# CobayaSampler/cobaya

Measured on AMD Instinct MI355X. Metric: log-posterior evals/sec (whole node), 30-dim gaussian_mixture, higher is better.
Workload: dtype f64

## Files before the change

cobaya_amd/csrc/capi.hip:

```cpp
#include "ctx.h"
#include "host_linalg.h"

int block_slots(const mcmc_hip_ctx* h, int which)
{
    if (!h->blocked) return h->d;
    int L = 0;
    for (size_t b = 0; b < h->blk_size.size(); ++b) {
        if (which == 0) L += h->blk_over[b] * h->blk_size[b];
        else if (which == 1) L += ((int)b <= h->drag_last_slow) ? h->blk_size[b] : 0;
        else L += ((int)b > h->drag_last_slow) ? h->blk_size[b] : 0;
    }
    return L;
}

int upload_constants(mcmc_hip_ctx* h)
{
    if (!h->have_prior || !h->have_target) return MCMC_HIP_OK;
    const int d = h->d, K = h->K;
    const ConstLayout cl{d, K};
    std::vector<double> c((size_t)cl.size() + 16, 0.0);
    for (int i = 0; i < d; ++i) {
        c[cl.lo() + i] = h->lo[i];
        c[cl.hi() + i] = h->hi[i];
        c[cl.loc() + i] = h->loc[i];
// ... 47 lines not shown
        if (K > 0) HIP_TRY(h, h->y.resize((size_t)K * d * h->W));
        if (K > 1) HIP_TRY(h, h->amode.resize((size_t)K * h->W));
        h->amode_valid = false;
        std::vector<double> pr((size_t)5 * dpad, 0.0);
        for (int i = 0; i < dpad; ++i) {
            pr[i] = i < d ? h->lo[i] : -INFINITY;
            pr[dpad + i] = i < d ? h->hi[i] : INFINITY;
            pr[2 * dpad + i] = i < d ? h->loc[i] : 0.0;
            const bool nrm = i < d && h->kind[i] == 1;
            pr[3 * dpad + i] = nrm ? 1.0 / h->scale[i] : 0.0;
            pr[4 * dpad + i] = nrm ? h->mls[i] : 0.0;
        }
        HIP_TRY(h, h->inc_prior.resize(pr.size()));
        HIP_TRY(h, hipMemcpyAsync(h->inc_prior.p, pr.data(), sizeof(double) * pr.size(),
                                  hipMemcpyHostToDevice, h->stream));
        if (K > 0) {
            HIP_TRY(h, h->inc_Lrow.resize((size_t)K * d * d));
            HIP_TRY(h, hipMemcpyAsync(h->inc_Lrow.p, h->Linv.data(), sizeof(double) * K * d * d,
                                      hipMemcpyHostToDevice, h->stream));
            HIP_TRY(h, h->inc_mean.resize((size_t)K * d));
            HIP_TRY(h, hipMemcpyAsync(h->inc_mean.p, h->mean.data(), sizeof(double) * K * d,
                                      hipMemcpyHostToDevice, h->stream));
        }
        h->y_valid = false; h->amode_valid = false;
    }
    HIP_TRY(h, hipStreamSynchronize(h->stream));
    return MCMC_HIP_OK;
}

namespace {

int lds_check(mcmc_hip_ctx* h)
{
    if (h->kb || h->huge) return MCMC_HIP_OK;
    const size_t lds = mcmc::step_lds_bytes(h->K, 256, h->gs, mcmc::v_slab(h->d));
    if (lds > mcmc::kLdsMax)
        return fail(h, MCMC_HIP_ERR_ARG,
                    "the step kernel needs %zu bytes of LDS per workgroup (> 160 KiB): fewer "
                    "mixture modes or a smaller group_size are required", lds);
    return MCMC_HIP_OK;
}

int set_target_common(mcmc_hip_ctx* h, int K, const double* means, const double* covs,
                      const double* weights, bool normalized)
{
    const int d = h->d;
    if (K < 1 || K > mcmc::kMaxModes)
// ... 193 lines not shown
        acc(h->nrows.resize(W));
    }
    acc(hipHostMalloc((void**)&h->pin_mom, sizeof(double) * (G * d + np + 2),
                      hipHostMallocCoherent | hipHostMallocMapped));
    if (h->pin_mom) acc(hipHostGetDevicePointer((void**)&h->pin_mom_dev, h->pin_mom, 0));
    acc(hipHostMalloc((void**)&h->pin_T, sizeof(double) * 4 * d * d, hipHostMallocDefault));
    for (auto& e : h->pin_T_done) acc(hipEventCreateWithFlags(&e, hipEventDisableTiming));
    acc(hipEventCreateWithFlags(&h->mom_event, hipEventDisableTiming));
    if (h->incremental) {
        int prio_least = 0, prio_greatest = 0;
        acc(hipDeviceGetStreamPriorityRange(&prio_least, &prio_greatest));
        acc(hipStreamCreateWithPriority(&h->stream2, hipStreamNonBlocking, prio_least));
        acc(hipEventCreateWithFlags(&h->mark, hipEventDisableTiming));
        acc(hipEventCreateWithFlags(&h->T_event, hipEventDisableTiming));
        if (const char* e = getenv("MCMC_HIP_EAGER_DIRECTIONS")) h->lazy_dirs = !(e[0] && e[0] != '0');
        if (const char* e = getenv("MCMC_HIP_LOOKAHEAD")) h->lookahead = std::max(1, atoi(e));
        if (const char* e = getenv("MCMC_HIP_DUO")) h->duo = (e[0] && e[0] != '0') ? 1 : 0;
        if (const char* e = getenv("MCMC_HIP_ACCEPT_SLACK")) {
            const double v = strtod(e, nullptr);
            h->accept_slack = v < mcmc::kAcceptSlack ? mcmc::kAcceptSlack : v;
        }
        for (auto& D : h->dirs) acc(hipEventCreateWithFlags(&D.ready, hipEventDisableTiming));
        h->prefetch = !getenv("MCMC_HIP_NO_PREFETCH");
    }
    if (r == hipSuccess) r = hipMemsetAsync(h->gsum.p, 0, sizeof(double) * G * d, h->stream);
    if (r == hipSuccess) r = hipMemsetAsync(h->pooled.p, 0, sizeof(double) * np, h->stream);
    if (r == hipSuccess) r = hipMemsetAsync(h->dshift.p, 0, sizeof(double) * d, h->stream);
    if (r == hipSuccess) r = hipMemsetAsync(h->stuck.p, 0, sizeof(int), h->stream);
    if (r == hipSuccess) r = hipMemsetAsync(h->acc_total.p, 0, sizeof(unsigned long long), h->stream);
    if (r == hipSuccess) r = hipStreamSynchronize(h->stream);
    if (r != hipSuccess) {
        fail(nullptr, MCMC_HIP_ERR_DEVICE, "device allocation failed: %s", hipGetErrorString(r));
        mcmc_hip_destroy(h);
        return MCMC_HIP_ERR_DEVICE;
    }
    *out = h;
    return MCMC_HIP_OK;
}

void mcmc_hip_destroy(mcmc_hip_ctx* h)
{
    if (!h) return;
    (void)hipSetDevice(h->cfg.device);
    if (h->stream) (void)hipStreamSynchronize(h->stream);
    if (h->stream2) (void)hipStreamSynchronize(h->stream2);
    resolve_timing(h);
// ... 11 lines not shown
    h->cblock.release(); h->dT.release(); h->V.release(); h->rows.release(); h->gsum.release();
    h->Sg.release(); h->pooled.p = nullptr;  h->dshift.release(); h->ex.release(); h->elp.release();
    h->ell.release(); h->eder.release(); h->escratch.release(); h->dLrow.release();
    h->dLcol.release(); h->weight_i.release(); h->prej.release();
    h->burn.release(); h->stuck.release(); h->nrows.release(); h->nacc.release();
    h->acc_total.p = nullptr;
    h->dblk.release(); h->vflag.release(); h->vflag_f.release(); h->Vf.release(); h->drag_cs.release();
    for (auto& sl : h->slots)
        if (sl.p) (void)hipHostFree(sl.p);
    h->ck.ring.release(); h->ck.wsum.release(); h->ck.payload.release(); h->ck.ws.release();
    h->ck.out.release(); h->ck.acc_prev.release();
    h->bd.ring.release(); h->bd.bounds.release(); h->bd.payload.release();
    if (h->bd.pin) (void)hipHostFree(h->bd.pin);
    if (h->ck.pin_out) (void)hipHostFree(h->ck.pin_out);
    destroy_product(h->mg); destroy_product(h->ac); destroy_product(h->bf);
    destroy_product(h->evd); destroy_product(h->dv); destroy_product(h->imp);
    h->imp.hist.destroy();
    if (h->ck.ev) (void)hipEventDestroy(h->ck.ev);
    if (h->pin_mom) (void)hipHostFree(h->pin_mom);
    if (h->pin_T) (void)hipHostFree(h->pin_T);
    for (auto& e : h->pin_T_done) if (e) (void)hipEventDestroy(e);
    if (h->mom_event) (void)hipEventDestroy(h->mom_event);
    h->pack_out.release(); h->pack_off.release();
    h->y.release(); h->amode.release(); h->inc_prior.release(); h->inc_Lrow.release();
    h->inc_mean.release();
    {
        auto& B = h->bg;
        B.bjs.release(); B.es.release(); B.Afused.release();
        B.resp.release(); B.theta0.release(); B.Astream.release(); B.weights.release();
        B.X.release(); B.dbins.release(); B.delta.release(); B.trial.release(); B.lp_t.release();
        B.Ea.release(); B.psum.release(); B.epsum.release(); B.edelta.release(); B.etrial.release(); B.elp.release();
        B.echi2.release(); B.ecl.release(); B.eA.release();
    }
    h->fnt.points.release(); h->fnt.lp_t.release(); h->fnt.Ea.release(); h->fnt.ll_t.release();
    h->fnt.bad.release();
    h->mv.q.release();
    h->fnt.dinputs.release(); h->fnt.ll_new.release(); h->fnt.ll_c.release();
    h->fnt.epts.release(); h->fnt.ell.release();
    for (auto& b : h->fnt.pts) b.release();
    if (h->stream) (void)hipStreamDestroy(h->stream);
    delete h;
}

int mcmc_hip_set_prior(mcmc_hip_ctx* h, const int32_t* kind, const double* a, const double* b,
                       const int32_t* periodic)
{
    if (!h) return MCMC_HIP_ERR_ARG;
// ... 327 lines not shown
    HIP_TRY(h, hipMemcpyAsync(h->logpost.p, lpost.data(), sizeof(double) * W, hipMemcpyHostToDevice, s));
    HIP_TRY(h, hipMemcpyAsync(h->logprior.p, lp.data(), sizeof(double) * W, hipMemcpyHostToDevice, s));
    HIP_TRY(h, hipMemcpyAsync(h->loglike.p, ll.data(), sizeof(double) * W, hipMemcpyHostToDevice, s));
    HIP_TRY(h, hipMemcpyAsync(h->weight_i.p, ones.data(), sizeof(int) * W, hipMemcpyHostToDevice, s));
    HIP_TRY(h, hipMemcpyAsync(h->prej.p, zeros.data(), sizeof(int) * W, hipMemcpyHostToDevice, s));
    HIP_TRY(h, hipMemcpyAsync(h->burn.p, burn.data(), sizeof(int) * W, hipMemcpyHostToDevice, s));
    HIP_TRY(h, hipMemcpyAsync(h->nacc.p, z64.data(), sizeof(long long) * W, hipMemcpyHostToDevice, s));
    if (h->nrows.p)
        HIP_TRY(h, hipMemcpyAsync(h->nrows.p, zeros.data(), sizeof(int) * W, hipMemcpyHostToDevice, s));
    HIP_TRY(h, hipMemsetAsync(h->stuck.p, 0, sizeof(int), s));
    if (h->fnt.bad.p) HIP_TRY(h, hipMemsetAsync(h->fnt.bad.p, 0, sizeof(int), s));
    if (h->fnt.on && h->fnt.n_fn > 0) {
        auto& F = h->fnt;
        if (F.last_eval_n != (int)W) return fail(h, MCMC_HIP_ERR_STATE, "no component log-likelihoods of the state");
        HIP_TRY(h, hipMemcpyAsync(F.ll_c.p, F.last_eval.data(), sizeof(double) * F.n_fn * W, hipMemcpyHostToDevice, s));
        F.llc_valid = true;
    }
    HIP_TRY(h, hipMemsetAsync(h->acc_total.p, 0, sizeof(unsigned long long), s));
    if (h->thin_acc.p) HIP_TRY(h, hipMemsetAsync(h->thin_acc.p, 0, sizeof(int) * W, s));
    HIP_TRY(h, hipStreamSynchronize(s));
    h->step = 0;
    h->have_state = true;
    h->mv.checked = false; h->mv.broken = false;
    h->y_valid = false; h->amode_valid = false;
    return MCMC_HIP_OK;
}

int mcmc_hip_get_state(mcmc_hip_ctx* h, double* x, double* logpost, double* logprior,
                       double* loglike, int32_t* weight)
{
    if (!h) return MCMC_HIP_ERR_ARG;
    if (!h->have_state) return fail(h, MCMC_HIP_ERR_STATE, "no state: call set_state first");
    const size_t W = h->W, d = h->d;
    hipStream_t s = h->stream;
    HIP_TRY(h, hipSetDevice(h->cfg.device));
    std::vector<double> xt;
    if (x) {
        xt.resize(W * d);
        HIP_TRY(h, hipMemcpyAsync(xt.data(), h->x.p, sizeof(double) * W * d, hipMemcpyDeviceToHost, s));
    }
    if (logpost) HIP_TRY(h, hipMemcpyAsync(logpost, h->logpost.p, sizeof(double) * W, hipMemcpyDeviceToHost, s));
    if (logprior) HIP_TRY(h, hipMemcpyAsync(logprior, h->logprior.p, sizeof(double) * W, hipMemcpyDeviceToHost, s));
    if (loglike) HIP_TRY(h, hipMemcpyAsync(loglike, h->loglike.p, sizeof(double) * W, hipMemcpyDeviceToHost, s));
    if (weight) HIP_TRY(h, hipMemcpyAsync(weight, h->weight_i.p, sizeof(int) * W, hipMemcpyDeviceToHost, s));
    HIP_TRY(h, hipStreamSynchronize(s));
    if (x)
        for (size_t w = 0; w < W; ++w)
// ... 38 lines not shown
            return fail(h, MCMC_HIP_ERR_ARG, "walker %zu has a non-finite log-posterior", w);
        for (size_t i = 0; i < d; ++i) xt[i * W + w] = x[w * d + i];
    }
    HIP_TRY(h, hipMemcpy(h->x.p, xt.data(), sizeof(double) * W * d, hipMemcpyHostToDevice));
    HIP_TRY(h, hipMemcpy(h->logpost.p, logpost, sizeof(double) * W, hipMemcpyHostToDevice));
    HIP_TRY(h, hipMemcpy(h->logprior.p, logprior, sizeof(double) * W, hipMemcpyHostToDevice));
    HIP_TRY(h, hipMemcpy(h->loglike.p, loglike, sizeof(double) * W, hipMemcpyHostToDevice));
    HIP_TRY(h, hipMemcpy(h->weight_i.p, weight, sizeof(int) * W, hipMemcpyHostToDevice));
    HIP_TRY(h, hipMemcpy(h->prej.p, prior_rej, sizeof(int) * W, hipMemcpyHostToDevice));
    HIP_TRY(h, hipMemcpy(h->burn.p, burn_left, sizeof(int) * W, hipMemcpyHostToDevice));
    HIP_TRY(h, hipMemcpy(h->nacc.p, n_accept, sizeof(int64_t) * W, hipMemcpyHostToDevice));
    if (h->nrows.p) HIP_TRY(h, hipMemset(h->nrows.p, 0, sizeof(int) * W));
    HIP_TRY(h, hipMemset(h->stuck.p, 0, sizeof(int)));
    if (h->fnt.bad.p) HIP_TRY(h, hipMemset(h->fnt.bad.p, 0, sizeof(int)));
    h->fnt.llc_valid = false;
    {
        unsigned long long tot = 0;
        for (size_t w = 0; w < W; ++w) tot += (unsigned long long)n_accept[w];
        HIP_TRY(h, hipMemcpy(h->acc_total.p, &tot, sizeof tot, hipMemcpyHostToDevice));
    }
    h->step = step;
    h->have_state = true;
    h->mv.checked = false; h->mv.broken = false;
    h->y_valid = false; h->amode_valid = false;
    return MCMC_HIP_OK;
}

namespace {
mcmc::ScratchShape scratch_shape_of(mcmc_hip_ctx* h)
{
    mcmc::ScratchShape s;
    const bool drag = h->drag_last_slow >= 0;
    s.d = h->d; s.K = h->K; s.W = h->W; s.group_size = h->gs;
    s.any_normal = h->norm_mask4[0] || h->norm_mask4[1] || h->norm_mask4[2] || h->norm_mask4[3];
    s.any_periodic = h->any_periodic;
    s.emit = h->cfg.emit_capacity > 0; s.emit_thin = h->emit_thin > 1;
    s.unit_t = h->cfg.temperature == 1.0;
    s.own_basis = h->own_basis; s.blocked = h->blocked;
    s.n_drag = drag ? h->drag_steps : 0;
    s.cps = block_slots(h, drag ? 1 : 0);
    s.cps_f = drag ? block_slots(h, 2) : 0;
    s.lane_compiled = h->k != nullptr; s.big_dp = h->kb ? h->kb->dp : 0; s.pair_compiled = h->kp != nullptr;
    return s;
}
}

int mcmc_hip_scratch_choice(const mcmc_hip_scratch_shape* shape, mcmc_hip_scratch_answer* out)
// ... 202 lines not shown
    HIP_TRY(h, hipSetDevice(h->cfg.device));
    HIP_TRY(h, hipMemcpyAsync(h->dshift.p, h->shift.data(), sizeof(double) * h->d,
                              hipMemcpyHostToDevice, h->stream));
    if (changed && h->ac.ro.on()) {
        h->ac.held = h->ac.head = 0;
        std::fill(h->ac.n_pairs.begin(), h->ac.n_pairs.end(), (int64_t)0);
        HIP_TRY(h, hipMemsetAsync(h->ac.ro.slab, 0, h->ac.ro.bytes(), h->stream));
    }
    HIP_TRY(h, hipStreamSynchronize(h->stream));
    return MCMC_HIP_OK;
}

int mcmc_hip_accumulate_moments(mcmc_hip_ctx* h)
{
    if (!h) return MCMC_HIP_ERR_ARG;
    if (!h->have_state) return fail(h, MCMC_HIP_ERR_STATE, "no state");
    HIP_TRY(h, hipSetDevice(h->cfg.device));
    Timed t(h, 2);
    mcmc::MomentArgs a{};
    a.x = h->x.p; a.shift = h->dshift.p; a.group_sum = h->gsum.p; a.Sg = h->Sg.p;
    a.pooled = h->pooled.p; a.W = h->W; a.G = h->G;
    if (h->huge) HIP_TRY(h, mcmc_hip_launch_huge_moments(&a, h->gs, h->d, h->stream));
    else if (h->kb) HIP_TRY(h, h->kb->moments(a, h->gs, h->d, h->stream));
    else HIP_TRY(h, h->k->moments(a, h->gs, h->stream));
    h->n_snapshots += 1;
    return MCMC_HIP_OK;
}

int mcmc_hip_read_moments(mcmc_hip_ctx* h, int64_t* n_snapshots, double* group_sum,
                          double* pooled_S, int32_t reset)
{
    if (!h) return MCMC_HIP_ERR_ARG;
    HIP_TRY(h, hipSetDevice(h->cfg.device));
    HIP_TRY(h, hipStreamSynchronize(h->stream));
    if (h->stream2) HIP_TRY(h, hipStreamSynchronize(h->stream2));
    resolve_timing(h);
    const size_t d = h->d, G = h->G, np = d * (d + 1) / 2;
    if (n_snapshots) *n_snapshots = h->n_snapshots;
    if (group_sum)
        HIP_TRY(h, hipMemcpy(group_sum, h->gsum.p, sizeof(double) * G * d, hipMemcpyDeviceToHost));
    if (pooled_S) {
        std::vector<double> p(np);
        HIP_TRY(h, hipMemcpy(p.data(), h->pooled.p, sizeof(double) * np, hipMemcpyDeviceToHost));
        for (size_t i = 0; i < d; ++i)
            for (size_t j = 0; j <= i; ++j)
                pooled_S[i * d + j] = pooled_S[j * d + i] = p[i * (i + 1) / 2 + j];
    }
// ... 136 lines not shown
```

cobaya_amd/csrc/capi_incremental.hip:

```cpp
#include "ctx.h"

int blocked_basis(mcmc_hip_ctx* h, int which, unsigned long long c0, int ncyc, int L, size_t slab,
                  DevBuf<double>& V, DevBuf<int>& flag, bool& any_1d, hipStream_t st, bool shared_schedule)
{
    if (!st) st = h->stream;
    const int nb = (int)h->blk_size.size();
    any_1d = false;
    for (int b = 0; b < nb; ++b) {
        const bool in_seq = which == 0 || (which == 1) == (b <= h->drag_last_slow);
        any_1d = any_1d || (in_seq && h->blk_size[b] == 1);
    }
    HIP_TRY(h, V.resize((size_t)h->BG * ncyc * slab));
    if (any_1d) HIP_TRY(h, flag.resize((size_t)h->BG * ncyc * L));
    mcmc::BlockedBasisArgs b{};
    b.T = h->dT.p; b.V = V.p; b.vflag = any_1d ? flag.p : nullptr;
    b.block_size = h->dblk.p; b.oversample = h->dblk.p + nb; b.i_of_j = h->dblk.p + 2 * nb;
    b.n_blocks = nb; b.d = h->d; b.which = which; b.drag_last_slow = h->drag_last_slow;
    b.L = L; b.slab = (int)slab;
    b.ld = h->d;
    b.nmax = *std::max_element(h->blk_size.begin(), h->blk_size.end());
    b.group0 = h->cfg.walker_offset / (uint32_t)h->bgs;
    b.cycle0 = (uint32_t)c0;
    b.key0 = (uint32_t)h->cfg.seed; b.key1 = (uint32_t)(h->cfg.seed >> 32);
    b.ncyc = ncyc;
// ... 282 lines not shown
    if (hit) return MCMC_HIP_OK;
    if (h->prefetch && h->lazy_dirs && h->mark_valid && h->stream2) {
        HIP_TRY(h, hipStreamWaitEvent(h->stream2, h->mark, 0));
        if (h->T_fresh) HIP_TRY(h, hipStreamWaitEvent(h->stream2, h->T_event, 0));
        const int rc = make_directions(h, C, P, span, D, h->stream2);
        if (rc != MCMC_HIP_OK) return rc;
        wait_ready = true;
    } else {
        const int rc = make_directions(h, C, P, span, D, h->stream);
        if (rc != MCMC_HIP_OK) return rc;
    }
    h->T_fresh = false;
    return MCMC_HIP_OK;
}

int launch_segment(mcmc_hip_ctx* h, const IncChoice& C, const IncPlan& P, mcmc_hip_ctx::DirSet& D,
                   bool inside, int room, bool& wait_ready, int& n)
{
    bool anchor = false;
    bool refresh_in_kernel = false;
    if (!h->y_valid || h->step % P.R == 0) {
        if (C.fold && inside) {
            refresh_in_kernel = true;
        } else {
            HIP_TRY(h, mcmc_hip_launch_whiten_state(h->x.p, h->y.p, h->inc_mean.p, h->inc_Lrow.p,
                                                    P.d, h->W, P.K, h->stream));
        }
        h->y_valid = true;
        anchor = true;
    }
    if (C.carry_modes && !h->amode_valid) anchor = true;
    n = plan_segment(P, h->step, room).n;
    if (wait_ready) {
        HIP_TRY(h, hipStreamWaitEvent(h->stream, D.ready, 0));
        wait_ready = false;
    }
    {
        Timed t(h, 0);
        const mcmc::IncStepArgs a =
            fill_inc_args(h, C, P, D, n, (anchor ? 1 : 0) | (refresh_in_kernel ? 2 : 0));
        if (C.carry_modes) h->amode_valid = true;
        HIP_TRY(h, P.launch(&a, h->stream));
        h->n_step_launches += 1;
        take_noted_kernel(h);
    }
    h->step += (unsigned long long)n;
    return MCMC_HIP_OK;
}

int prepare_next_set(mcmc_hip_ctx* h, const IncChoice& C, const IncPlan& P, int left, int n_steps)
{
    auto& N = h->dirs[h->dir_cur ^ 1];
    if (C.fold) {
// ... 54 lines not shown
    int left = n_steps;
    while (left > 0) {
        IncSeg span = plan_span(C, P, h->step, left);
        bool wait_ready = false;
        int rc = acquire_direction_set(h, C, P, span, false, wait_ready);
        if (rc != MCMC_HIP_OK) return rc;
        int n = 0;
        rc = launch_segment(h, C, P, h->dirs[h->dir_cur], false, span.n, wait_ready, n);
        if (rc != MCMC_HIP_OK) return rc;
        left -= n;
        rc = prepare_next_set(h, C, P, left, n_steps);
        if (rc != MCMC_HIP_OK) return rc;
    }
    return MCMC_HIP_OK;
}

}

mcmc::IncChoice inc_choice_of(const mcmc_hip_ctx* h)
{
    if (!h->incremental) return IncChoice{};
    const IncShape s = inc_shape_of(h);
    return mcmc::inc_choose(s, inc_any_fits(s, true));
}

int step_incremental(mcmc_hip_ctx* h, int n_steps)
{
    const int d = h->d, K = h->K;
    const IncShape S = inc_shape_of(h);
    const IncChoice C = mcmc::inc_choose(S, inc_any_fits(S, true));
    if (C.reason == mcmc::kIncBadShape || C.reason == mcmc::kIncDragShape)
        return fail(h, MCMC_HIP_ERR_ARG,
                    "incremental evaluation with dragging serves one Gaussian mode with "
                    "non-periodic priors; use evaluation: full for this model");
    if (C.reason == mcmc::kIncAnyLds)
        return fail(h, MCMC_HIP_ERR_ARG,
                    "incremental evaluation: %d modes at d=%d with %d periodic parameters do not "
                    "fit the LDS of a CU; use evaluation: full for this model", K, d, S.n_periodic);
    if (C.reason == mcmc::kIncEmitDrag && h->emit_thin > 1)
        return fail(h, MCMC_HIP_ERR_ARG,
                    "emit_thin: rows are thinned on the device by the incremental Metropolis kernels; "
                    "thin on the host");
    if (C.reason == mcmc::kIncEmitDrag)
        return fail(h, MCMC_HIP_ERR_ARG,
                    "incremental evaluation emits rows (emit_capacity > 0) with Metropolis "
                    "steps; use evaluation: full for dragging with emitted rows");
// ... 62 lines not shown
        h->y_valid = true;
    }
    HIP_TRY(h, hipStreamSynchronize(h->stream));
    const size_t W = h->W, d = (size_t)h->d * (size_t)h->K;
    std::vector<double> yt(W * d);
    HIP_TRY(h, hipMemcpy(yt.data(), h->y.p, sizeof(double) * W * d, hipMemcpyDeviceToHost));
    for (size_t w = 0; w < W; ++w)
        for (size_t i = 0; i < d; ++i) y[w * d + i] = yt[i * W + w];
    return MCMC_HIP_OK;
}

int mcmc_hip_set_whitened(mcmc_hip_ctx* h, const double* y)
{
    if (!h) return MCMC_HIP_ERR_ARG;
    if (!h->incremental || !y) return fail(h, MCMC_HIP_ERR_ARG, "not in incremental mode, or null");
    if (!h->have_state) return fail(h, MCMC_HIP_ERR_STATE, "set_full_state must precede set_whitened");
    HIP_TRY(h, hipSetDevice(h->cfg.device));
    HIP_TRY(h, hipStreamSynchronize(h->stream));
    const size_t W = h->W, d = (size_t)h->d * (size_t)h->K;
    std::vector<double> yt(W * d);
    for (size_t w = 0; w < W; ++w)
        for (size_t i = 0; i < d; ++i) yt[i * W + w] = y[w * d + i];
    HIP_TRY(h, hipMemcpy(h->y.p, yt.data(), sizeof(double) * W * d, hipMemcpyHostToDevice));
    h->y_valid = true;
    return MCMC_HIP_OK;
}

int mcmc_hip_incremental_carries_periodic(const mcmc_hip_ctx* h)
{
    return h && inc_choice_of(h).carry_periodic ? 1 : 0;
}

int mcmc_hip_accept_estimate_error(double* max_err, uint32_t* ka_at_max)
{
    if (!max_err || !ka_at_max) return MCMC_HIP_ERR_ARG;
    if (!mcmc_hip_launch_accept_estimate_error) return MCMC_HIP_ERR_ARG;
    constexpr int nb = 4096;
    double* derr = nullptr;
    uint32_t* dka = nullptr;
    std::vector<double> err(nb);
    std::vector<uint32_t> ka(nb);
    hipError_t r = hipMalloc(&derr, sizeof(double) * nb);
    if (r == hipSuccess) r = hipMalloc(&dka, sizeof(uint32_t) * nb);
    if (r == hipSuccess) r = mcmc_hip_launch_accept_estimate_error(derr, dka, nb, nullptr);
    if (r == hipSuccess) r = hipMemcpy(err.data(), derr, sizeof(double) * nb, hipMemcpyDeviceToHost);
    if (r == hipSuccess) r = hipMemcpy(ka.data(), dka, sizeof(uint32_t) * nb, hipMemcpyDeviceToHost);
    if (derr) (void)hipFree(derr);
// ... 52 lines not shown
```

cobaya_amd/csrc/ctx.h:

```cpp
#pragma once
#include "../../include/mcmc_hip.h"

#include <algorithm>
#include <cmath>
#include <cstdarg>
#include <cstdio>
#include <cstring>
#include <limits>
#include <string>
#include <vector>

#define MCMC_HIP_HOST_SIDE 1
#include "kernels.h"
#include "huge_args.h"
#include "pliklite_args.h"
#include "function_args.h"
#include "stretch_args.h"
#include "ensemble_move_args.h"
#include "checkpoint_args.h"
#include "marginal_args.h"
#include "autocorr_args.h"
#include "bestfit_args.h"
#include "evidence_args.h"
#include "derived_args.h"
// ... 112 lines not shown
    bool have_prior = false, have_target = false, have_cov = false, have_state = false;
    std::vector<int32_t> kind, periodic;
    std::vector<double> lo, hi, loc, scale, mls;
    double uniform_logp = 0.0;
    uint32_t norm_mask = 0, periodic_mask = 0;
    uint32_t norm_mask4[4] = {0, 0, 0, 0};
    bool any_periodic = false;
    std::vector<double> mean, Linv, cnorm, weight;
    std::vector<double> cov, T;
    bool blocked = false;
    std::vector<int32_t> blk_size, blk_over, i_of_j;
    int drag_last_slow = -1, drag_steps = 0;
    DevBuf<int> dblk, vflag, vflag_f;
    DevBuf<double> Vf;
    DevBuf<double> drag_cs;
    std::vector<double> shift;
    DevBuf<double> x, logpost, logprior, loglike, cblock, dT, V, rows, gsum, Sg, pooled, dshift;
    DevBuf<double> ex, elp, ell, eder, escratch, dLrow, dLcol;
    bool incremental = false;
    bool y_valid = false;
    bool own_basis = false;
    int bgs = 0, BG = 0;
    DevBuf<double> y, inc_prior, inc_Lrow, inc_mean;
    DevBuf<double> amode;
    bool amode_valid = false;
    struct DirSet {
        DevBuf<double> V, Vf, VU;
        DevBuf<int> vflag, vflag_f, colflag;
        bool has_flags = false;
        DevBuf<double> UU;
        DevBuf<double> VW, NL;
        hipEvent_t ready = nullptr;
        bool ahead = false;
        unsigned long long step0 = ~0ull, epoch = 0;
        int n = 0;
    } dirs[2];
    int dir_cur = 0;
    unsigned long long dir_epoch = 0;
    hipStream_t stream2 = nullptr;
    hipEvent_t mark = nullptr;
    bool mark_valid = false;
    bool prefetch = true;
    bool lazy_dirs = true;
    int lookahead = 4;
    size_t dir_budget = 0;
    int duo = -1;
// ... 349 lines not shown
int step_functions(mcmc_hip_ctx* h, int n_steps);
int functions_evaluate(mcmc_hip_ctx* h, int n, const double* x, double* comps);
int evaluate_binned_points(mcmc_hip_ctx* h, int n, const double* x, double* logprior, double* loglike);
int function_call(mcmc_hip_ctx* h, int n, const double* points, double* loglike);
int function_target_error(mcmc_hip_ctx* h, int bad);
inline uint32_t philox_w0(uint32_t k0, uint32_t k1, uint32_t c0, uint32_t c1, uint32_t c2, uint32_t c3)
{
    for (int r = 0; r < 10; ++r) {
        const uint64_t p0 = (uint64_t)0xD2511F53u * c0, p1 = (uint64_t)0xCD9E8D57u * c2;
        const uint32_t n0 = (uint32_t)(p1 >> 32) ^ c1 ^ k0, n2 = (uint32_t)(p0 >> 32) ^ c3 ^ k1;
        c0 = n0; c1 = (uint32_t)p1; c2 = n2; c3 = (uint32_t)p0;
        k0 += 0x9E3779B9u; k1 += 0xBB67AE85u;
    }
    return c0;
}

int step_stretch(mcmc_hip_ctx* h, int n_steps);
int blocked_basis(mcmc_hip_ctx* h, int which, unsigned long long c0, int ncyc, int L, size_t slab,
                  DevBuf<double>& V, DevBuf<int>& flag, bool& any_1d, hipStream_t st = nullptr,
                  bool shared_schedule = false);
int step_huge(mcmc_hip_ctx* h, int n_steps);
int step_incremental(mcmc_hip_ctx* h, int n_steps);
mcmc::IncChoice inc_choice_of(const mcmc_hip_ctx* h);
```

cobaya_amd/csrc/incremental_kernels.hip:

```cpp
#include <string>

#include "incremental_common.h"

#ifndef MCMC_INC_DMA_HIDDEN
#define MCMC_INC_DMA_HIDDEN(dq, mode) ((dq) >= 25 && (mode) == 0)
#endif

namespace mcmc {
namespace {

__host__ __device__ constexpr bool inc_one_wave_regs(int dq, int mode, bool per)
{
    return !per && ((mode == 1 && dq >= 31) || (mode == 2 && dq >= 32));
}

__host__ __device__ constexpr int inc_min_waves(int dq, int mode, bool per = false)
{
    if (per) return MCMC_EXP_WAVES(STEP, dq <= 8 ? 4 : dq <= 31 ? 2 : 1);
    return MCMC_EXP_WAVES(STEP,
        mode == 0 ? (dq <= 12 ? 4 : dq <= 30 ? 2 : 1)
        : mode == 1 ? ((dq <= 8 || dq == 13) ? 4 : dq <= 30 ? 2 : 1)
        : (dq <= 8 ? 4 : dq <= 31 ? 2 : 1));
}

__host__ __device__ constexpr bool inc_bounds_in_lds(int dq, int mode, bool per)
// ... 831 lines not shown
                x0[kk] = sel(accept_m, ce[kk], x0[kk]);
                y0[kk] = sel(accept_m, ye[kk], y0[kk]);
            }
        }
        asm volatile("s_waitcnt vmcnt(0)" ::: "memory");
        __syncthreads();
    }
#pragma unroll
    for (int kk = 0; kk < DQ; ++kk) {
        const int i = 4 * kk + c;
        if (i < d) {
            s.x[(size_t)i * W + w] = x0[kk];
            a.y[(size_t)i * W + w] = y0[kk];
        }
    }
    if (c == 0) {
        s.logpost[w] = lpost; s.logprior[w] = lpri; s.loglike[w] = llik;
        s.weight[w] = wt; s.prior_rej[w] = prej; s.burn_left[w] = burn;
        s.n_accept[w] = nacc;
    }
    wave_add_accepts(s.accept_total, (c == 0) ? nacc - nacc0 : 0);
}

template <int NR>
__device__ __forceinline__ void rows_times_column(cdoubles L, int d, int j0,
                                                  const double* __restrict__ col, double (&acc)[NR])
{
    cdoubles r[NR];
#pragma unroll
    for (int q = 0; q < NR; ++q) { r[q] = L + (size_t)(j0 + q) * d; acc[q] = 0.0; }
    int i = 0;
    for (; i + 8 <= j0; i += 8) {
        double c[8], m[NR][8];
#pragma unroll
        for (int u = 0; u < 8; ++u) {
            c[u] = col[(i + u) * 64];
#pragma unroll
            for (int q = 0; q < NR; ++q) m[q][u] = r[q][i + u];
        }
#pragma unroll
        for (int u = 0; u < 8; ++u)
#pragma unroll
            for (int q = 0; q < NR; ++q) acc[q] = fma(m[q][u], c[u], acc[q]);
    }
    if (i < j0) {
        double c[4], m[NR][4];
#pragma unroll
        for (int u = 0; u < 4; ++u) {
            c[u] = col[(i + u) * 64];
#pragma unroll
            for (int q = 0; q < NR; ++q) m[q][u] = r[q][i + u];
        }
#pragma unroll
        for (int u = 0; u < 4; ++u)
#pragma unroll
            for (int q = 0; q < NR; ++q) acc[q] = fma(m[q][u], c[u], acc[q]);
    }
    double c[NR], m[NR][NR];
#pragma unroll
    for (int u = 0; u < NR; ++u) {
        c[u] = col[(j0 + u) * 64];
#pragma unroll
        for (int q = u; q < NR; ++q) m[q][u] = r[q][j0 + u];
    }
#pragma unroll
    for (int u = 0; u < NR; ++u)
#pragma unroll
        for (int q = u; q < NR; ++q) acc[q] = fma(m[q][u], c[u], acc[q]);
}

template <class Put>
__device__ __forceinline__ void row_blocks_times_column(cdoubles L, int d, int part,
                                                        const double* __restrict__ col, Put&& put)
{
    const int nblk = (d + 3) / 4;
    for (int pr = part; 2 * pr < nblk; pr += 4) {
        for (int s = 0; s < 2; ++s) {
            const int rb = s ? nblk - 1 - pr : pr;
            if (s && rb == pr) break;
            const int j0 = 4 * rb, nr = d - j0;
            if (nr >= 4) {
                double acc[4];
                rows_times_column<4>(L, d, j0, col, acc);
                put(j0, acc[0]); put(j0 + 1, acc[1]); put(j0 + 2, acc[2]); put(j0 + 3, acc[3]);
            } else if (nr == 3) {
                double acc[3];
                rows_times_column<3>(L, d, j0, col, acc);
                put(j0, acc[0]); put(j0 + 1, acc[1]); put(j0 + 2, acc[2]);
            } else if (nr == 2) {
                double acc[2];
                rows_times_column<2>(L, d, j0, col, acc);
                put(j0, acc[0]); put(j0 + 1, acc[1]);
            } else {
                double acc[1];
                rows_times_column<1>(L, d, j0, col, acc);
                put(j0, acc[0]);
            }
        }
    }
}

__global__ void __launch_bounds__(256) whiten_state_kernel(const double* __restrict__ x,
                                                           double* __restrict__ y,
                                                           const double* __restrict__ mean,
                                                           const double* __restrict__ Lrow, int d,
                                                           int W, int K)
{
    extern __shared__ __attribute__((aligned(16))) double sdev[];
    const int l = threadIdx.x & 63, part = __builtin_amdgcn_readfirstlane(threadIdx.x >> 6),
              w = blockIdx.x * 64 + l;
    const bool live = w < W;
    for (int k = 0; k < K; ++k) {
        __syncthreads();
        if (live) {
            for (int i0 = part; i0 < d; i0 += 32) {
                double xv[8];
#pragma unroll
                for (int u = 0; u < 8; ++u) {
                    const int i = i0 + 4 * u;
                    xv[u] = i < d ? x[(size_t)i * W + w] : 0.0;
                }
#pragma unroll
                for (int u = 0; u < 8; ++u) {
// ... 756 lines not shown
```

cobaya_amd/csrc/kernels.h:

```cpp
#pragma once
#include <hip/hip_runtime.h>
#include <stdint.h>

#include "inc_choice.h"
#include "scratch_choice.h"

namespace mcmc {

__host__ __device__ constexpr int tri_size(int d) { return d * (d + 1) / 2; }

template <typename F>
__host__ __device__ inline void tri_stream_for_each(int d, F&& f)
{
    int idx = 0;
    for (int jb = 0; jb < d; jb += kRowBlock)
        for (int i = 0; i < jb + kRowBlock && i < d; ++i)
            for (int r = 0; r < kRowBlock; ++r)
                if (jb + r < d && i <= jb + r) f(idx++, jb + r, i);
}

struct ConstLayout {
    int d, K;
    __host__ __device__ int lo() const { return 0; }
    __host__ __device__ int hi() const { return d; }
// ... 78 lines not shown
struct EvalArgs {
    const double* x;
    double* logprior;
    double* loglike;
    double* derived;
    const double* cblock;
    int n;
    int n_modes;
    uint32_t norm_mask, periodic_mask;
    uint32_t norm_mask4[4];
    double uniform_logp;
};

struct MomentArgs {
    const double* x;
    const double* shift;
    double* group_sum;
    double* Sg;
    double* pooled;
    int W;
    int G;
};

struct DragArgs {
    StepArgs s;
    const double* Vf;
    const int* vflag_f;
    unsigned long long cyc0, cyc0_f;
    int cps_f, slab_f, ncyc_f;
    int n_drag;
};

struct DimKernels {
    hipError_t (*step)(const StepArgs&, const ScratchChoice&, hipStream_t);
    hipError_t (*basis)(const BasisArgs&, int n_groups, hipStream_t);
    hipError_t (*evaluate)(const EvalArgs&, hipStream_t);
    hipError_t (*moments)(const MomentArgs&, int group_size, hipStream_t);
    hipError_t (*drag)(const DragArgs&, const ScratchChoice&, hipStream_t);
};

typedef hipError_t (*PairStep)(const StepArgs*, const ScratchChoice*, hipStream_t);

struct GeneralStepArgs {
    StepArgs s;
    const double* Lrow;
    int d;
    uint32_t norm_mask4[4];
    uint32_t periodic_mask4[4];
    int ld;
    int own_basis;
};

struct GeneralDragArgs {
    GeneralStepArgs g;
    const double* Vf;
    const int* vflag_f;
    double* cs;
    unsigned long long cyc0, cyc0_f;
    int cps_f, slab_f, ncyc_f;
    int n_drag;
};
// ... 107 lines not shown
```

cobaya_amd/csrc/walker_kernels.hip:

```cpp
#include "det_math.h"
#include "kernels.h"

#ifndef MCMC_CH
#define MCMC_CH 16
#endif
#ifndef MCMC_D
#error "compile with -DMCMC_D=<dimension>"
#endif

namespace mcmc {
namespace {

constexpr int D = MCMC_D;
constexpr int NPAIR = D * (D + 1) / 2;
constexpr bool kBigD = D > kMaxDimLane;
constexpr int LDV = kBigD ? v_ld(D) : D;

typedef const double __attribute__((address_space(4))) * cptr;
__device__ __forceinline__ cptr as_const(const double* p) { return (cptr)(unsigned long long)p; }
__device__ __forceinline__ cptr launder(cptr p)
{
    unsigned long long v = (unsigned long long)p;
    asm volatile("; operand base of this step" : "+s"(v));
    return (cptr)v;
// ... 1100 lines not shown
{
    extern __shared__ __attribute__((aligned(16))) double sA[];
    const ConstLayout cl{D, a.n_modes};
    const cptr C = as_const(a.cblock);
    const int tid = threadIdx.x;
    const int p = blockIdx.x * 64 + tid;
    if (p >= a.n) return;
    double t[D];
#pragma unroll
    for (int i = 0; i < D; ++i) t[i] = a.x[(size_t)p * D + i];
    bool inb;
    double lp, ll;
    double* der = DERIVED ? a.derived + (size_t)p * (cl.K > 0 ? cl.K : 1) * D : nullptr;
    eval_point<MULTI, DERIVED, true>(t, C, cl, a.norm_mask, a.uniform_logp, sA + tid, 64, inb, lp,
                                     ll, der);
    a.logprior[p] = inb ? lp : -INFINITY;
    a.loglike[p] = inb ? ll : -INFINITY;
}

constexpr int kMomNb = (D + 1) / 2;
constexpr int kMomLd = (2 * kMomNb) % 4 == 2 ? 2 * kMomNb : 2 * kMomNb + 2;
constexpr int kMomTiles = kMomNb * (kMomNb + 1) / 2;

__global__ void __launch_bounds__(256) group_moments_kernel(const MomentArgs a)
{
    extern __shared__ __attribute__((aligned(16))) double sX[];
    const int tid = threadIdx.x, gs = blockDim.x, g = blockIdx.x;
    const int w = g * gs + tid;
    {
        double xv[2 * kMomNb];
#pragma unroll
        for (int i = 0; i < 2 * kMomNb; ++i) xv[i] = i < D ? a.x[(size_t)i * a.W + w] : 0.0;
        double2* __restrict__ row = (double2*)(sX + tid * kMomLd);
#pragma unroll
        for (int k = 0; k < kMomNb; ++k)
            row[k] = make_double2(xv[2 * k] - a.shift[2 * k],
                                  2 * k + 1 < D ? xv[2 * k + 1] - a.shift[2 * k + 1] : 0.0);
    }
    __syncthreads();
    constexpr int B = 8;
    for (int t = tid; t < kMomTiles; t += gs) {
        int I = (int)((sqrtf(8.0f * (float)t + 1.0f) - 1.0f) * 0.5f);
        while ((I + 1) * (I + 2) / 2 <= t) ++I;
        while (I * (I + 1) / 2 > t) --I;
        const int J = t - I * (I + 1) / 2;
        const double2* __restrict__ pa = (const double2*)(sX + 2 * I);
        const double2* __restrict__ pb = (const double2*)(sX + 2 * J);
        double s00 = 0.0, s01 = 0.0, s10 = 0.0, s11 = 0.0;
        double2 A[2][B], Bv[2][B];
#pragma unroll
// ... 25 lines not shown
        const int i0 = 2 * I, j0 = 2 * J, i1 = i0 + 1, j1 = j0 + 1;
        Sg[i0 * (i0 + 1) / 2 + j0] = s00;
        if (I != J) Sg[i0 * (i0 + 1) / 2 + j1] = s01;
        if (i1 < D) {
            Sg[i1 * (i1 + 1) / 2 + j0] = s10;
            if (j1 < D) Sg[i1 * (i1 + 1) / 2 + j1] = s11;
        }
    }
    if ((tid >> 6) == (gs >> 6) - 1) {
        for (int k = tid & 63; k < kMomNb; k += 64) {
            const double2* __restrict__ pa = (const double2*)(sX + 2 * k);
            double s0 = 0.0, s1 = 0.0;
            for (int l = 0; l < gs; l += B) {
                double2 v[B];
#pragma unroll
                for (int q = 0; q < B; ++q) v[q] = pa[(l + q) * (kMomLd / 2)];
#pragma unroll
                for (int q = 0; q < B; ++q) { s0 = s0 + v[q].x; s1 = s1 + v[q].y; }
            }
            a.group_sum[(size_t)g * D + 2 * k] += s0;
            if (2 * k + 1 < D) a.group_sum[(size_t)g * D + 2 * k + 1] += s1;
        }
    }
}

__global__ void __launch_bounds__(64) pool_moments_kernel(const MomentArgs a)
{
    const int p = blockIdx.x * 64 + threadIdx.x;
    if (p >= NPAIR) return;
    double acc = a.pooled[p];
    int g = 0;
    for (; g + 64 <= a.G; g += 64) {
        double v[64];
#pragma unroll
        for (int u = 0; u < 64; ++u) v[u] = a.Sg[(size_t)(g + u) * NPAIR + p];
#pragma unroll
        for (int u = 0; u < 64; ++u) acc += v[u];
    }
    for (; g + 16 <= a.G; g += 16) {
        double v[16];
#pragma unroll
        for (int u = 0; u < 16; ++u) v[u] = a.Sg[(size_t)(g + u) * NPAIR + p];
#pragma unroll
        for (int u = 0; u < 16; ++u) acc += v[u];
    }
    for (; g < a.G; ++g) acc += a.Sg[(size_t)g * NPAIR + p];
// ... 53 lines not shown
    const bool multi = a.n_modes > 1;
    const size_t lds = sizeof(double) * (size_t)(multi ? a.n_modes * 64 : 0);
    const dim3 grid((a.n + 63) / 64), block(64);
    if (multi) {
        if (a.derived) hipLaunchKernelGGL((evaluate_kernel<true, true>), grid, block, lds, st, a);
        else hipLaunchKernelGGL((evaluate_kernel<true, false>), grid, block, lds, st, a);
    } else {
        if (a.derived) hipLaunchKernelGGL((evaluate_kernel<false, true>), grid, block, lds, st, a);
        else hipLaunchKernelGGL((evaluate_kernel<false, false>), grid, block, lds, st, a);
    }
    return hipGetLastError();
}

hipError_t launch_moments(const MomentArgs& a, int group_size, hipStream_t st)
{
    if (group_size <= 0 || group_size > 256 || group_size % 64 != 0)
        return hipErrorInvalidValue;
    const size_t lds = sizeof(double) * (size_t)group_size * kMomLd;
    hipLaunchKernelGGL(group_moments_kernel, dim3(a.G), dim3(group_size), lds, st, a);
    hipLaunchKernelGGL(pool_moments_kernel, dim3((NPAIR + 63) / 64), dim3(64), 0, st, a);
    return hipGetLastError();
}

hipError_t launch_drag(const DragArgs& a, const ScratchChoice& c, hipStream_t st)
{
    typedef void (*kern_t)(const DragArgs);
    const kern_t kern = c.multi ? drag_kernel<true> : drag_kernel<false>;
    if (c.lds_attr) {
        hipError_t e = hipFuncSetAttribute((const void*)kern, hipFuncAttributeMaxDynamicSharedMemorySize,
                                           (int)c.lds_attr);
        if (e != hipSuccess) return e;
    }
    mcmc_hip_note_step_kernel(c.multi ? "mcmc::drag_kernel<true>" : "mcmc::drag_kernel<false>");
    hipLaunchKernelGGL(kern, dim3(c.grid), dim3(c.threads), c.lds_bytes, st, a);
    return hipGetLastError();
}

const DimKernels kKernels = {launch_step, launch_basis, launch_evaluate, launch_moments,
                             launch_drag};
#endif

}
}

#define MCMC_CAT2(a, b) a##b
#define MCMC_CAT(a, b) MCMC_CAT2(a, b)
#if MCMC_D <= 32
extern "C" const mcmc::DimKernels* MCMC_CAT(mcmc_hip_dim_, MCMC_D)() { return &mcmc::kKernels; }
#else
static_assert(MCMC_D <= mcmc::kMaxDimPair, "two-wave kernel: d <= kMaxDimPair");
extern "C" hipError_t MCMC_CAT(mcmc_hip_pair_, MCMC_D)(const mcmc::StepArgs* a, const mcmc::ScratchChoice* c,
                                                      hipStream_t st)
{
    return mcmc::launch_pair(*a, *c, st);
}
#endif
```

Measured before the change: 103.5 billion.

## Fuse whitening of walker state into the snapshot moments kernel launch

When a moments snapshot lands on a whitening-refresh step, one launch now computes group moments and also whitens the state into a look-ahead y buffer, using extra blocks. The next incremental step swaps that buffer in instead of launching a separate whiten_state kernel. This is meant to save a separate launch and a re-read of x, at the cost of an extra K*d*W device buffer and more invalidation bookkeeping. The shared row-block matrix-vector helper is generalized to handle several waves and moved to a header.

```diff
diff --git a/cobaya_amd/csrc/capi.hip b/cobaya_amd/csrc/capi.hip
--- a/cobaya_amd/csrc/capi.hip
+++ b/cobaya_amd/csrc/capi.hip
@@ -93,7 +93,7 @@
             HIP_TRY(h, hipMemcpyAsync(h->inc_mean.p, h->mean.data(), sizeof(double) * K * d,
                                       hipMemcpyHostToDevice, h->stream));
         }
-        h->y_valid = false; h->amode_valid = false;
+        h->y_valid = false; h->y_ahead_ok = false; h->amode_valid = false;
     }
     HIP_TRY(h, hipStreamSynchronize(h->stream));
     return MCMC_HIP_OK;
@@ -333,6 +333,7 @@
         }
         for (auto& D : h->dirs) acc(hipEventCreateWithFlags(&D.ready, hipEventDisableTiming));
         h->prefetch = !getenv("MCMC_HIP_NO_PREFETCH");
+        if (const char* e = getenv("MCMC_HIP_FUSED_SNAPSHOT")) h->fused_snapshot = !(e[0] == '0' && !e[1]);
     }
     if (r == hipSuccess) r = hipMemsetAsync(h->gsum.p, 0, sizeof(double) * G * d, h->stream);
     if (r == hipSuccess) r = hipMemsetAsync(h->pooled.p, 0, sizeof(double) * np, h->stream);
@@ -390,7 +391,7 @@
     for (auto& e : h->pin_T_done) if (e) (void)hipEventDestroy(e);
     if (h->mom_event) (void)hipEventDestroy(h->mom_event);
     h->pack_out.release(); h->pack_off.release();
-    h->y.release(); h->amode.release(); h->inc_prior.release(); h->inc_Lrow.release();
+    h->y.release(); h->y_ahead.release(); h->amode.release(); h->inc_prior.release(); h->inc_Lrow.release();
     h->inc_mean.release();
     {
         auto& B = h->bg;
@@ -764,7 +765,7 @@
     h->step = 0;
     h->have_state = true;
     h->mv.checked = false; h->mv.broken = false;
-    h->y_valid = false; h->amode_valid = false;
+    h->y_valid = false; h->y_ahead_ok = false; h->amode_valid = false;
     return MCMC_HIP_OK;
 }
 
@@ -849,7 +850,7 @@
     h->step = step;
     h->have_state = true;
     h->mv.checked = false; h->mv.broken = false;
-    h->y_valid = false; h->amode_valid = false;
+    h->y_valid = false; h->y_ahead_ok = false; h->amode_valid = false;
     return MCMC_HIP_OK;
 }
 
@@ -1098,7 +1099,14 @@
     a.pooled = h->pooled.p; a.W = h->W; a.G = h->G;
     if (h->huge) HIP_TRY(h, mcmc_hip_launch_huge_moments(&a, h->gs, h->d, h->stream));
     else if (h->kb) HIP_TRY(h, h->kb->moments(a, h->gs, h->d, h->stream));
-    else HIP_TRY(h, h->k->moments(a, h->gs, h->stream));
+    else if (snapshot_forms_y(h)) {
+        HIP_TRY(h, h->y_ahead.resize((size_t)h->K * h->d * h->W));
+        mcmc::WhitenArgs wa{};
+        wa.y = h->y_ahead.p; wa.mean = h->inc_mean.p; wa.Lrow = h->inc_Lrow.p; wa.K = h->K;
+        HIP_TRY(h, h->k->moments_whiten(a, wa, h->gs, h->stream));
+        h->y_ahead_ok = true;
+        h->y_ahead_step = h->step;
+    } else HIP_TRY(h, h->k->moments(a, h->gs, h->stream));
     h->n_snapshots += 1;
     return MCMC_HIP_OK;
 }
diff --git a/cobaya_amd/csrc/capi_incremental.hip b/cobaya_amd/csrc/capi_incremental.hip
--- a/cobaya_amd/csrc/capi_incremental.hip
+++ b/cobaya_amd/csrc/capi_incremental.hip
@@ -328,6 +328,8 @@
     if (!h->y_valid || h->step % P.R == 0) {
         if (C.fold && inside) {
             refresh_in_kernel = true;
+        } else if (h->y_ahead_ok && h->y_ahead_step == h->step) {
+            std::swap(h->y, h->y_ahead);
         } else {
             HIP_TRY(h, mcmc_hip_launch_whiten_state(h->x.p, h->y.p, h->inc_mean.p, h->inc_Lrow.p,
                                                     P.d, h->W, P.K, h->stream));
@@ -335,6 +337,7 @@
         h->y_valid = true;
         anchor = true;
     }
+    h->y_ahead_ok = false;
     if (C.carry_modes && !h->amode_valid) anchor = true;
     n = plan_segment(P, h->step, room).n;
     if (wait_ready) {
@@ -435,6 +438,18 @@
     if (!h->incremental) return IncChoice{};
     const IncShape s = inc_shape_of(h);
     return mcmc::inc_choose(s, inc_any_fits(s, true));
+}
+
+bool snapshot_forms_y(const mcmc_hip_ctx* h)
+{
+    if (!h->fused_snapshot || !h->incremental || h->huge || !h->k || !h->k->moments_whiten) return false;
+    if (!h->have_target || !h->have_state || !h->y_valid || h->K < 1 || !h->inc_Lrow.p || !h->inc_mean.p) return false;
+    if (h->bg.on || h->fnt.on || h->mv.kind == MCMC_HIP_MOVE_STRETCH || h->mx.n > 0) return false;
+    if (h->gs % 64 != 0 || h->gs > 256 || h->W != h->G * h->gs) return false;
+    const IncChoice C = inc_choice_of(h);
+    if (C.family == mcmc::kIncNotServed) return false;
+    const unsigned long long R = 40ull * (unsigned long long)block_slots(h, C.drag() ? 1 : 0);
+    return R > 0 && h->step % R == 0;
 }
 
 int step_incremental(mcmc_hip_ctx* h, int n_steps)
@@ -543,7 +558,7 @@
     for (size_t w = 0; w < W; ++w)
         for (size_t i = 0; i < d; ++i) yt[i * W + w] = y[w * d + i];
     HIP_TRY(h, hipMemcpy(h->y.p, yt.data(), sizeof(double) * W * d, hipMemcpyHostToDevice));
-    h->y_valid = true;
+    h->y_valid = true; h->y_ahead_ok = false;
     return MCMC_HIP_OK;
 }
 
diff --git a/cobaya_amd/csrc/ctx.h b/cobaya_amd/csrc/ctx.h
--- a/cobaya_amd/csrc/ctx.h
+++ b/cobaya_amd/csrc/ctx.h
@@ -158,6 +158,10 @@
     bool own_basis = false;
     int bgs = 0, BG = 0;
     DevBuf<double> y, inc_prior, inc_Lrow, inc_mean;
+    DevBuf<double> y_ahead;
+    bool y_ahead_ok = false;
+    unsigned long long y_ahead_step = 0;
+    bool fused_snapshot = true;
     DevBuf<double> amode;
     bool amode_valid = false;
     struct DirSet {
@@ -553,3 +557,4 @@
 int step_huge(mcmc_hip_ctx* h, int n_steps);
 int step_incremental(mcmc_hip_ctx* h, int n_steps);
 mcmc::IncChoice inc_choice_of(const mcmc_hip_ctx* h);
+bool snapshot_forms_y(const mcmc_hip_ctx* h);
diff --git a/cobaya_amd/csrc/incremental_kernels.hip b/cobaya_amd/csrc/incremental_kernels.hip
--- a/cobaya_amd/csrc/incremental_kernels.hip
+++ b/cobaya_amd/csrc/incremental_kernels.hip
@@ -1,6 +1,7 @@
 #include <string>
 
 #include "incremental_common.h"
+#include "whiten_rows.h"
 
 #ifndef MCMC_INC_DMA_HIDDEN
 #define MCMC_INC_DMA_HIDDEN(dq, mode) ((dq) >= 25 && (mode) == 0)
@@ -878,83 +879,6 @@
     wave_add_accepts(s.accept_total, (c == 0) ? nacc - nacc0 : 0);
 }
 
-template <int NR>
-__device__ __forceinline__ void rows_times_column(cdoubles L, int d, int j0,
-                                                  const double* __restrict__ col, double (&acc)[NR])
-{
-    cdoubles r[NR];
-#pragma unroll
-    for (int q = 0; q < NR; ++q) { r[q] = L + (size_t)(j0 + q) * d; acc[q] = 0.0; }
-    int i = 0;
-    for (; i + 8 <= j0; i += 8) {
-        double c[8], m[NR][8];
-#pragma unroll
-        for (int u = 0; u < 8; ++u) {
-            c[u] = col[(i + u) * 64];
-#pragma unroll
-            for (int q = 0; q < NR; ++q) m[q][u] = r[q][i + u];
-        }
-#pragma unroll
-        for (int u = 0; u < 8; ++u)
-#pragma unroll
-            for (int q = 0; q < NR; ++q) acc[q] = fma(m[q][u], c[u], acc[q]);
-    }
-    if (i < j0) {
-        double c[4], m[NR][4];
-#pragma unroll
-        for (int u = 0; u < 4; ++u) {
-            c[u] = col[(i + u) * 64];
-#pragma unroll
-            for (int q = 0; q < NR; ++q) m[q][u] = r[q][i + u];
-        }
-#pragma unroll
-        for (int u = 0; u < 4; ++u)
-#pragma unroll
-            for (int q = 0; q < NR; ++q) acc[q] = fma(m[q][u], c[u], acc[q]);
-    }
-    double c[NR], m[NR][NR];
-#pragma unroll
-    for (int u = 0; u < NR; ++u) {
-        c[u] = col[(j0 + u) * 64];
-#pragma unroll
-        for (int q = u; q < NR; ++q) m[q][u] = r[q][j0 + u];
-    }
-#pragma unroll
-    for (int u = 0; u < NR; ++u)
-#pragma unroll
-        for (int q = u; q < NR; ++q) acc[q] = fma(m[q][u], c[u], acc[q]);
-}
-
-template <class Put>
-__device__ __forceinline__ void row_blocks_times_column(cdoubles L, int d, int part,
-                                                        const double* __restrict__ col, Put&& put)
-{
-    const int nblk = (d + 3) / 4;
-    for (int pr = part; 2 * pr < nblk; pr += 4) {
-        for (int s = 0; s < 2; ++s) {
-            const int rb = s ? nblk - 1 - pr : pr;
-            if (s && rb == pr) break;
-            const int j0 = 4 * rb, nr = d - j0;
-            if (nr >= 4) {
-                double acc[4];
-                rows_times_column<4>(L, d, j0, col, acc);
-                put(j0, acc[0]); put(j0 + 1, acc[1]); put(j0 + 2, acc[2]); put(j0 + 3, acc[3]);
-            } else if (nr == 3) {
-                double acc[3];
-                rows_times_column<3>(L, d, j0, col, acc);
-                put(j0, acc[0]); put(j0 + 1, acc[1]); put(j0 + 2, acc[2]);
-            } else if (nr == 2) {
-                double acc[2];
-                rows_times_column<2>(L, d, j0, col, acc);
-                put(j0, acc[0]); put(j0 + 1, acc[1]);
-            } else {
-                double acc[1];
-                rows_times_column<1>(L, d, j0, col, acc);
-                put(j0, acc[0]);
-            }
-        }
-    }
-}
 
 __global__ void __launch_bounds__(256) whiten_state_kernel(const double* __restrict__ x,
                                                            double* __restrict__ y,
diff --git a/cobaya_amd/csrc/kernels.h b/cobaya_amd/csrc/kernels.h
--- a/cobaya_amd/csrc/kernels.h
+++ b/cobaya_amd/csrc/kernels.h
@@ -124,6 +124,13 @@
     int G;
 };
 
+struct WhitenArgs {
+    double* y;
+    const double* mean;
+    const double* Lrow;
+    int K;
+};
+
 struct DragArgs {
     StepArgs s;
     const double* Vf;
@@ -139,6 +146,7 @@
     hipError_t (*evaluate)(const EvalArgs&, hipStream_t);
     hipError_t (*moments)(const MomentArgs&, int group_size, hipStream_t);
     hipError_t (*drag)(const DragArgs&, const ScratchChoice&, hipStream_t);
+    hipError_t (*moments_whiten)(const MomentArgs&, const WhitenArgs&, int group_size, hipStream_t);
 };
 
 typedef hipError_t (*PairStep)(const StepArgs*, const ScratchChoice*, hipStream_t);
diff --git a/cobaya_amd/csrc/walker_kernels.hip b/cobaya_amd/csrc/walker_kernels.hip
--- a/cobaya_amd/csrc/walker_kernels.hip
+++ b/cobaya_amd/csrc/walker_kernels.hip
@@ -1,5 +1,6 @@
 #include "det_math.h"
 #include "kernels.h"
+#include "whiten_rows.h"
 
 #ifndef MCMC_CH
 #define MCMC_CH 16
@@ -1146,10 +1147,9 @@
 constexpr int kMomLd = (2 * kMomNb) % 4 == 2 ? 2 * kMomNb : 2 * kMomNb + 2;
 constexpr int kMomTiles = kMomNb * (kMomNb + 1) / 2;
 
-__global__ void __launch_bounds__(256) group_moments_kernel(const MomentArgs a)
-{
-    extern __shared__ __attribute__((aligned(16))) double sX[];
-    const int tid = threadIdx.x, gs = blockDim.x, g = blockIdx.x;
+__device__ __forceinline__ void group_moments_block(const MomentArgs& a, double* sX, const int g)
+{
+    const int tid = threadIdx.x, gs = blockDim.x;
     const int w = g * gs + tid;
     {
         double xv[2 * kMomNb];
@@ -1221,6 +1221,46 @@
             if (2 * k + 1 < D) a.group_sum[(size_t)g * D + 2 * k + 1] += s1;
         }
     }
+}
+
+__global__ void __launch_bounds__(256) group_moments_kernel(const MomentArgs a)
+{
+    extern __shared__ __attribute__((aligned(16))) double sX[];
+    group_moments_block(a, sX, blockIdx.x);
+}
+
+template <int NW>
+__device__ __forceinline__ void whiten_group_block(const MomentArgs& a, const WhitenArgs& wa, double* sdev, const int g)
+{
+    constexpr int gs = 64 * NW;
+    const int tid = threadIdx.x, l = tid & 63, part = __builtin_amdgcn_readfirstlane(tid >> 6);
+    const size_t w0 = (size_t)g * gs;
+    double xv[D];
+#pragma unroll
+    for (int i = 0; i < D; ++i) xv[i] = a.x[(size_t)i * a.W + w0 + tid];
+    for (int k = 0; k < wa.K; ++k) {
+        if (k) __syncthreads();
+#pragma unroll
+        for (int i = 0; i < D; ++i) sdev[i * gs + tid] = xv[i] - wa.mean[k * D + i];
+        __syncthreads();
+        const cdoubles L = (cdoubles)(unsigned long long)(wa.Lrow + (size_t)k * D * D);
+        double* __restrict__ out = wa.y + (size_t)k * D * a.W + w0 + l;
+        row_blocks_times_columns<NW, NW>(L, D, part, sdev + l, gs,
+                                         [&](int j, int s, double v) { out[(size_t)j * a.W + s * 64] = v; });
+    }
+}
+
+__global__ void __launch_bounds__(256) snapshot_whiten_kernel(const MomentArgs a, const WhitenArgs wa)
+{
+    extern __shared__ __attribute__((aligned(16))) double sX[];
+    if ((int)blockIdx.x < a.G) {
+        group_moments_block(a, sX, blockIdx.x);
+        return;
+    }
+    const int g = (int)blockIdx.x - a.G;
+    if (blockDim.x == 256) whiten_group_block<4>(a, wa, sX, g);
+    else if (blockDim.x == 128) whiten_group_block<2>(a, wa, sX, g);
+    else whiten_group_block<1>(a, wa, sX, g);
 }
 
 __global__ void __launch_bounds__(64) pool_moments_kernel(const MomentArgs a)
@@ -1320,6 +1360,16 @@
     return hipGetLastError();
 }
 
+hipError_t launch_moments_whiten(const MomentArgs& a, const WhitenArgs& wa, int group_size, hipStream_t st)
+{
+    if ((group_size != 64 && group_size != 128 && group_size != 256) || a.W != a.G * group_size || wa.K < 1)
+        return hipErrorInvalidValue;
+    const size_t lds = sizeof(double) * (size_t)group_size * kMomLd;
+    hipLaunchKernelGGL(snapshot_whiten_kernel, dim3(2 * a.G), dim3(group_size), lds, st, a, wa);
+    hipLaunchKernelGGL(pool_moments_kernel, dim3((NPAIR + 63) / 64), dim3(64), 0, st, a);
+    return hipGetLastError();
+}
+
 hipError_t launch_drag(const DragArgs& a, const ScratchChoice& c, hipStream_t st)
 {
     typedef void (*kern_t)(const DragArgs);
@@ -1335,7 +1385,7 @@
 }
 
 const DimKernels kKernels = {launch_step, launch_basis, launch_evaluate, launch_moments,
-                             launch_drag};
+                             launch_drag, launch_moments_whiten};
 #endif
 
 }
diff --git a/cobaya_amd/csrc/whiten_rows.h b/cobaya_amd/csrc/whiten_rows.h
--- /dev/null
+++ b/cobaya_amd/csrc/whiten_rows.h
@@ -0,0 +1,111 @@
+#pragma once
+
+namespace mcmc {
+namespace {
+
+typedef const double __attribute__((address_space(4))) * cdoubles;
+
+template <int NR, int NW>
+__device__ __forceinline__ void rows_times_columns(cdoubles L, int d, int j0, const double* __restrict__ col,
+                                                   int ld, double (&acc)[NW][NR])
+{
+    cdoubles r[NR];
+#pragma unroll
+    for (int q = 0; q < NR; ++q) {
+        r[q] = L + (size_t)(j0 + q) * d;
+#pragma unroll
+        for (int s = 0; s < NW; ++s) acc[s][q] = 0.0;
+    }
+    int i = 0;
+    for (; i + 8 <= j0; i += 8) {
+        double c[NW][8], m[NR][8];
+#pragma unroll
+        for (int u = 0; u < 8; ++u) {
+#pragma unroll
+            for (int s = 0; s < NW; ++s) c[s][u] = col[(i + u) * ld + s * 64];
+#pragma unroll
+            for (int q = 0; q < NR; ++q) m[q][u] = r[q][i + u];
+        }
+#pragma unroll
+        for (int u = 0; u < 8; ++u)
+#pragma unroll
+            for (int q = 0; q < NR; ++q)
+#pragma unroll
+                for (int s = 0; s < NW; ++s) acc[s][q] = fma(m[q][u], c[s][u], acc[s][q]);
+    }
+    if (i < j0) {
+        double c[NW][4], m[NR][4];
+#pragma unroll
+        for (int u = 0; u < 4; ++u) {
+#pragma unroll
+            for (int s = 0; s < NW; ++s) c[s][u] = col[(i + u) * ld + s * 64];
+#pragma unroll
+            for (int q = 0; q < NR; ++q) m[q][u] = r[q][i + u];
+        }
+#pragma unroll
+        for (int u = 0; u < 4; ++u)
+#pragma unroll
+            for (int q = 0; q < NR; ++q)
+#pragma unroll
+                for (int s = 0; s < NW; ++s) acc[s][q] = fma(m[q][u], c[s][u], acc[s][q]);
+    }
+    double c[NW][NR], m[NR][NR];
+#pragma unroll
+    for (int u = 0; u < NR; ++u) {
+#pragma unroll
+        for (int s = 0; s < NW; ++s) c[s][u] = col[(j0 + u) * ld + s * 64];
+#pragma unroll
+        for (int q = u; q < NR; ++q) m[q][u] = r[q][j0 + u];
+    }
+#pragma unroll
+    for (int u = 0; u < NR; ++u)
+#pragma unroll
+        for (int q = u; q < NR; ++q)
+#pragma unroll
+            for (int s = 0; s < NW; ++s) acc[s][q] = fma(m[q][u], c[s][u], acc[s][q]);
+}
+
+template <int NPARTS, int NW, class Put>
+__device__ __forceinline__ void row_blocks_times_columns(cdoubles L, int d, int part, const double* __restrict__ col,
+                                                         int ld, Put&& put)
+{
+    const int nblk = (d + 3) / 4;
+    for (int pr = part; 2 * pr < nblk; pr += NPARTS) {
+        for (int h = 0; h < 2; ++h) {
+            const int rb = h ? nblk - 1 - pr : pr;
+            if (h && rb == pr) break;
+            const int j0 = 4 * rb, nr = d - j0;
+            if (nr >= 4) {
+                double acc[NW][4];
+                rows_times_columns<4, NW>(L, d, j0, col, ld, acc);
+#pragma unroll
+                for (int s = 0; s < NW; ++s) { put(j0, s, acc[s][0]); put(j0 + 1, s, acc[s][1]); put(j0 + 2, s, acc[s][2]); put(j0 + 3, s, acc[s][3]); }
+            } else if (nr == 3) {
+                double acc[NW][3];
+                rows_times_columns<3, NW>(L, d, j0, col, ld, acc);
+#pragma unroll
+                for (int s = 0; s < NW; ++s) { put(j0, s, acc[s][0]); put(j0 + 1, s, acc[s][1]); put(j0 + 2, s, acc[s][2]); }
+            } else if (nr == 2) {
+                double acc[NW][2];
+                rows_times_columns<2, NW>(L, d, j0, col, ld, acc);
+#pragma unroll
+                for (int s = 0; s < NW; ++s) { put(j0, s, acc[s][0]); put(j0 + 1, s, acc[s][1]); }
+            } else {
+                double acc[NW][1];
+                rows_times_columns<1, NW>(L, d, j0, col, ld, acc);
+#pragma unroll
+                for (int s = 0; s < NW; ++s) put(j0, s, acc[s][0]);
+            }
+        }
+    }
+}
+
+template <class Put>
+__device__ __forceinline__ void row_blocks_times_column(cdoubles L, int d, int part,
+                                                        const double* __restrict__ col, Put&& put)
+{
+    row_blocks_times_columns<4, 1>(L, d, part, col, 64, [&](int j, int, double v) { put(j, v); });
+}
+
+}
+}
```

Result: no change. 104.0 billion, median of 6 (+0.6%).
